# tobwei/APTAI

Hardware: AMD Instinct MI355X
Metric: utterances/sec (10 s @ 16 kHz) train-step (higher is better)
Workload: dtype bf16

## Files before the change

aptai_amd/_lib.py:

```python
from __future__ import annotations

import ctypes
import os
import subprocess
import threading

import torch

_HERE = os.path.dirname(os.path.abspath(__file__))
CSRC = os.path.join(_HERE, "csrc")
LIB_PATH = os.environ.get("APTAI_HIP_LIB") or os.path.join(CSRC, "libaptai_hip.so")

_lib = None
_lock = threading.Lock()

_P, _I64, _I, _F, _U64 = ctypes.c_void_p, ctypes.c_int64, ctypes.c_int, ctypes.c_float, ctypes.c_uint64
ARGTYPES = {
    "aptai_layernorm_fwd": [_P, _P, _P, _P, _P, _P, _I64, _I64, _F, _I, _P],
    "aptai_layernorm_bwd": [_P, _P, _P, _P, _P, _P, _P, _P, _F, _U64, _P, _P, _P, _I64, _I64, _P, _P],
    "aptai_layernorm_bwd_workspace_bytes": [_I64, _I64],
    "aptai_layernorm_bwd_finalize_multi": [_P, _I64, _I64, _P],
    "aptai_layernorm_fwd_f32in": [_P, _P, _P, _P, _P, _I64, _I64, _F, _P],
    "aptai_layernorm_fwd_f32in_split": [_P, _P, _P, _P, _P, _I, _I64, _I64, _F, _P],
    "aptai_attention_fwd": [_P, _P, _P, _P, _P, _I64, _I64, _I64, _I64, _F, _F, _U64, _I, _P],
    "aptai_attention_bwd": [_P, _P, _P, _P, _P, _P, _P, _P, _I64, _I64, _I64, _I64, _F, _F, _U64, _I, _I, _P],
    "aptai_attention_probs_fwd": [_P, _P, _P, _P, _I64, _I64, _I64, _I64, _F, _F, _U64, _I, _P],
    "aptai_attention_probs_bwd": [_P, _P, _P, _P, _P, _P, _I64, _I64, _I64, _I64, _F, _F, _U64, _I, _I, _P],
    "aptai_cast_f32_to_bf16": [_P, _P, _I64, _I64, _I64, _P],
    "aptai_conv_weight_to_bf16": [_P, _P, _I64, _I64, _I64, _P],
    "aptai_posconv_weight": [_P, _P, _P, _P, _P, _I64, _I64, _I64, _P],
    "aptai_posconv_pack": [_P, _P, _P, _P, _I64, _I64, _I64, _I64, _I64, _P],
    "aptai_frame_mask_fwd": [_P, _P, _P, _P, _I64, _I64, _I64, _I64, _P],
    "aptai_frame_mask_bwd": [_P, _P, _P, _P, _P, _I64, _I64, _I64, _I64, _P],
    "aptai_frame_mask_bwd_workspace_bytes": [_I64, _I64, _I64],
    "aptai_colsum_bf16": [_P, _I64, _P, _P, _I64, _I64, _I, _P],
    "aptai_colsum_workspace_bytes": [_I64, _I64],
    "aptai_dropout_bf16": [_P, _P, _I64, _F, _U64, _P],
    "aptai_dgelu_bf16": [_P, _P, _P, _I64, _P],
    "aptai_conv0_fwd": [_P, _I64, _I64, _P, _P, _P, _P, _I, _F, _P, _I64, _I64, _I64, _I64, _I64, _P, _P, _P],
    "aptai_conv0_bwd": [_P, _I64, _I64, _P, _P, _P, _P, _I, _F, _P, _I64, _I64, _P, _P, _P, _P, _P, _P, _P],
    "aptai_conv0_bwd_workspace_bytes": [_I64, _I64],
    "aptai_conv0_bwd_data": [_P, _I64, _I64, _P, _P, _P, _P, _I, _F, _P, _I64, _I64, _P, _P, _P, _P],
    "aptai_conv0_bwd_data_workspace_bytes": [_I64, _I64],
    "aptai_conv0_workspace_bytes": [_I64, _I64],
    "aptai_head_act_fwd": [_P, _P, _P, _I64, _F, _F, _U64, _P],
    "aptai_head_act_bwd": [_P, _P, _P, _P, _I64, _F, _F, _U64, _P],
    "aptai_lowpass_fir": [_P, _I64, _I64, _P, _I64, _P, _I64, _I64, _I, _I64, _I64, _I64, _I64, _I64, _P],
    "aptai_aptai_loss_fwd": [_P, _P, _P, _I64, _I64, _P, _I64, _I64, _I64, _I64, _F, _F, _P, _P, _P, _P],
    "aptai_aptai_loss_bwd": [_P, _P, _P, _I64, _I64, _P, _I64, _I64, _I64, _I64, _F, _F, _P, _P, _P, _P, _I64, _P],
    "aptai_aptai_loss_workspace_bytes": [],
    "aptai_gemm_workspace_bytes": [_I64, _I64, _I],
    "aptai_gemm_sk_workspace_bytes": [],
    "aptai_gemm_sk_status": [_P, _P, _P],
    "aptai_cast_multi": [_P, _I64, _I64, _P],
    "aptai_posconv_weight_bwd": [_P, _P, _P, _P, _P, _P, _P, _I64, _I64, _I64, _P],
    "aptai_spec_augment_mask": [_P, _P, _I64, _I64, _F, _I64, _I64, _U64, _P],
    "aptai_posconv_wgrad": [_P, _P, _P, _I64, _I64, _I64, _I64, _I64, _I64, _P],
    "aptai_posconv_gemm": [_P, _I64, _P, _P, _P, _P, _P, _I64, _I64, _I64, _I64, _I64, _I64, _I, _P],
    "aptai_adam_multi": [_P, _P, _I64, _I64, _F, _F, _F, _F, _F, _P],
    "aptai_sgemm_f32": [_P, _I, _I64, _I64, _P, _I64, _I64, _P, _I64, _P, _F, _I, _I64, _I64, _I64, _I64, _I64, _I64, _I64, _I64, _P, _P],
    "aptai_sgemm_workspace_bytes": [_I64, _I64, _I64, _I64],
    "aptai_colsum_f32_workspace_bytes": [_I64],
    "aptai_embed_pe_fwd": [_P, _P, _P, _P, _I64, _I64, _I64, _F, _U64, _P],
    "aptai_embed_bwd": [_P, _P, _P, _I64, _I64, _F, _U64, _P],
    "aptai_xattn_softmax_fwd": [_P, _P, _P, _P, _P, _P, _P, _I64, _I64, _I64, _P],
    "aptai_xattn_softmax_bwd": [_P, _P, _P, _P, _I64, _P, _I64, _I64, _P],
    "aptai_layernorm_f32_fwd": [_P, _P, _P, _P, _P, _P, _I64, _I64, _F, _P],
    "aptai_layernorm_f32_bwd": [_P, _P, _P, _P, _P, _P, _P, _P, _P, _I64, _I64, _P],
    "aptai_layernorm_f32_bwd_workspace_bytes": [_I64],
    "aptai_lstm_fwd": [_P, _P, _P, _P, _P, _P, _P, _I64, _I64, _I64, _I64, _P],
    "aptai_lstm_bwd": [_P, _P, _P, _P, _P, _P, _P, _I64, _I64, _I64, _I64, _P],
    "aptai_lstm_workspace_bytes": [_I64],
    "aptai_lstm_fwd_serial": [_P, _P, _P, _P, _P, _P, _I64, _I64, _I64, _I64, _P],
    "aptai_lstm_bwd_serial": [_P, _P, _P, _P, _P, _P, _I64, _I64, _I64, _I64, _P],
    "aptai_gather_alignment": [_P, _P, _P, _P, _I64, _I64, _I64, _P],
    "aptai_tanh_dropout_f32": [_P, _P, _P, _P, _I64, _F, _U64, _P],
    "aptai_dropout_f32": [_P, _P, _I64, _F, _U64, _P],
    "aptai_colsum_f32": [_P, _I64, _P, _P, _I64, _I64, _P],
    "aptai_ctc_fwd": [_P, _I64, _I64, _P, _I64, _P, _P, _P, _I64, _I64, _I64, _I, _I, _I, _P, _P, _P, _P, _I, _P],
    "aptai_ctc_bwd": [_P, _I64, _I64, _P, _I64, _P, _P, _P, _I64, _I64, _I64, _I, _I, _I, _P, _P, _P, _F, _P, _I64, _I, _I, _P],
    "aptai_ctc_workspace_bytes": [_I64, _I64, _I64],
    "aptai_ctc_viterbi": [_P, _I64, _I64, _P, _I64, _P, _P, _P, _I64, _I64, _I64, _I, _I, _P, _P, _P, _P, _P, _P],
    "aptai_ctc_viterbi_workspace_bytes": [_I64, _I64, _I64],
    "aptai_ctc_greedy_decode": [_P, _I64, _I64, _I64, _I64, _I64, _I, _P, _I64, _P, _P],
    "aptai_mx_quantize_bf16": [_P, _I64, _P, _I64, _P, _I64, _I64, _I64, _P],
    "aptai_gemm_mxfp8": [_P, _P, _I64, _I64, _P, _P, _I64, _I64, _P, _I64, _P, _I, _P, _I64, _I64, _I64, _I64, _P],
    "aptai_layernorm_fwd_mx": [_P, _P, _P, _P, _P, _I64, _P, _I64, _I64, _I64, _F, _P],
    "aptai_gemm_mxfp8_mxout": [_P, _P, _I64, _I64, _P, _P, _I64, _I64, _P, _I64, _P, _I64, _P, _I, _I64, _I64, _I64, _P],
    "aptai_split_f32": [_P, _I64, _I64, _I64, _I, _I, _I, _P, _I64, _P],
    "aptai_bias_act_res_f32": [_P, _I64, _P, _P, _I64, _P, _I64, _I64, _I64, _I, _P, _I64, _P],
    "aptai_softmax_rows_f32": [_P, _P, _I64, _I64, _I64, _P],
    "aptai_softmax_split_f32": [_P, _P, _I64, _I64, _I64, _I, _P, _I64, _P],
    "aptai_attention_exact_fwd": [_P, _I64, _P, _P, _I64, _I64, _I64, _I64, _I64, _I, _F, _P],
    "aptai_conv0_fwd_f32": [_P, _I64, _I64, _P, _P, _P, _P, _I, _F, _P, _I64, _I64, _P, _P],
    "aptai_conv0_fwd_split": [_P, _I64, _I64, _P, _P, _P, _P, _I, _F, _P, _I, _I64, _I64, _P, _P],
    "aptai_device_check": [ctypes.c_char_p, _I],
    "aptai_set_seed_salt": [_P, _P],
    "aptai_set_frame_bounds": [_P, _P],
}


class AptaiHipError(RuntimeError):
    pass


def build(force: bool = False, jobs: int = 8) -> str:
# ... 43 lines not shown
```

aptai_amd/csrc/gemm.hip:

```cpp
#include <stdlib.h>

#include <mutex>
#include <set>

#include "common.h"
#include "gemm_common.h"

using namespace aptai_gemm;

namespace {

#ifdef APTAI_STAMPS
__device__ unsigned long long g_stamps[4096 * 8];
#define APTAI_STAMP(slot)                                                                          \
    do {                                                                                           \
        if (threadIdx.x == 0 && blockIdx.x < 4096 && blockIdx.y == 0 && blockIdx.z == 0)           \
            g_stamps[blockIdx.x * 8 + (slot)] = wall_clock64();                                    \
    } while (0)
extern "C" int aptai_debug_read_stamps(void* host_out) {
    return hipMemcpyFromSymbol(host_out, HIP_SYMBOL(g_stamps), sizeof(g_stamps)) == hipSuccess ? 0 : 1;
}
#else
#define APTAI_STAMP(slot) do {} while (0)
#endif

void epi_trace(const GemmArgs& g, int tile) {
    static const bool on = getenv("APTAI_EPI_TRACE") != nullptr;
    if (!on) return;
    static std::mutex mu;
    static std::set<int> seen;
    const int w = g.flags | (g.out_pre ? EPX_PRE : 0) | (g.colscale_n > 0 ? EPX_CS : 0);
    std::lock_guard<std::mutex> lk(mu);
    if (!seen.insert(w).second) return;
    bool listed = false;
#define APTAI_EPI_CASE(W) listed = listed || (w == (W));
    APTAI_EPI_WORDS(APTAI_EPI_CASE)
#undef APTAI_EPI_CASE
    fprintf(stderr, "[aptai epi] flag word 0x%x (tile %d, %d x %d x %d): %s\n", w, tile, g.M, g.N, g.K, listed ? "compiled" : "RUN-TIME form");
}

template <bool A_KM, bool B_KM, bool OUT_F32, int BM_T = 128>
__device__ __forceinline__ void gemm_tile_body(GemmArgs g, const int bid, const int batch, const int split) {
    extern __shared__ __attribute__((aligned(16))) char smem[];
    APTAI_STAMP(0);
    const int tid = threadIdx.x;
    const int lane = tid & 63;
    const int wave = __builtin_amdgcn_readfirstlane(tid >> 6);
    const int wm = wave >> 1, wn = wave & 1;

    int tile_m, tile_n;
    raster2d(bid, g.tiles_m, g.tiles_n, g.raster_gm, tile_m, tile_n);
    constexpr int NI = BM_T / 32;
    constexpr int WM = BM_T / 2;
    constexpr int NA_IT = BM_T / 32;
    constexpr int A_BYTES_T = BM_T * BK * 2;
    constexpr int STAGE_T = A_BYTES_T + BN * BK * 2;
    constexpr int NPASS = BM_T / 16;
    static_assert(BM_T == 128 || (BM_T == 64 && !A_KM), "64-row tiles are built for K-contiguous A only");
    constexpr bool RING5 = A_KM && B_KM && BM_T == 128 && APTAI_GEMM_RING5;
// ... 316 lines not shown
                const int m = m0_e + pass * 16 + (tid_e >> 4);
                const bool ok = n_ok && m < g.M;
                u32x4 rq = {0u, 0u, 0u, 0u}, aq = {0u, 0u, 0u, 0u};
                if (ok && (flags & APTAI_EPI_RESIDUAL)) rq = *(const u32x4*)(g.residual + (long)m * g.ldr + n);
                if (ok && (flags & (APTAI_EPI_DGELU | APTAI_EPI_MUL_AUX))) aq = *(const u32x4*)(g.aux + (long)m * g.ldaux + n);
                one_pass(pass, aq, rq);
            }
        } else {
#pragma unroll
            for (int pass = 0; pass < NPASS; ++pass) {
                one_pass(pass, auxv[PREF ? pass : 0], resv[PREF ? pass : 0]);
                asm volatile("" ::: "memory");
            }
        }
    };
    if (OUT_F32) body(EpiWord<-1>{});
    else epi_dispatch(fx, body);
    APTAI_STAMP(3);
#ifdef APTAI_STAMPS
    asm volatile("s_waitcnt vmcnt(0)" ::: "memory");
    APTAI_STAMP(4);
#endif
}

template <bool A_KM, bool B_KM, bool OUT_F32>
__global__ __launch_bounds__(NTHREADS, 3) void gemm_kernel(GemmArgs g) {
#ifdef APTAI_EXP_STAGGER
    if (g.exp_sleep > 0) {
        bool late = true;
        if (g.exp_cu_count != nullptr) {
            unsigned hwid, xcc;
            asm volatile("s_getreg_b32 %0, hwreg(HW_REG_HW_ID)" : "=s"(hwid));
            asm volatile("s_getreg_b32 %0, hwreg(HW_REG_XCC_ID)" : "=s"(xcc));
            __shared__ unsigned arrival;
            if (threadIdx.x == 0) arrival = atomicAdd(g.exp_cu_count + ((xcc & 7u) * 256u + ((hwid >> 8) & 0xffu)), 1u);
            __syncthreads();
            late = arrival == 1u;
        }
        if (late) for (int i = 0; i < g.exp_sleep; ++i) __builtin_amdgcn_s_sleep(31);
    }
#endif
    gemm_tile_body<A_KM, B_KM, OUT_F32>(g, xcd_remap(blockIdx.x, g.tiles_m * g.tiles_n), gridDim.y > 1 ? (int)blockIdx.y : -1,
                                        blockIdx.z);
}

constexpr int SMEM_M64_BYTES = 2 * (64 + BN) * BK * 2;
template <bool B_KM, bool OUT_F32>
__global__ __launch_bounds__(NTHREADS, 3) void gemm_kernel_m64(GemmArgs g) {
    gemm_tile_body<false, B_KM, OUT_F32, 64>(g, xcd_remap(blockIdx.x, g.tiles_m * g.tiles_n), gridDim.y > 1 ? (int)blockIdx.y : -1,
                                             blockIdx.z);
}

constexpr int MAX_GROUP = 8;
struct GroupArgs {
    GemmArgs p[MAX_GROUP];
    int tile_end[MAX_GROUP];
    int n, total;
};

template <bool A_KM, bool B_KM, bool OUT_F32>
__global__ __launch_bounds__(NTHREADS, 3) void gemm_grouped_kernel(GroupArgs ga) {
    const int bid = xcd_remap(blockIdx.x, ga.total);
    int pi = 0;
#pragma unroll
    for (int i = 1; i < MAX_GROUP; ++i)
        if (i < ga.n && bid >= ga.tile_end[i - 1]) pi = i;
    const int first = pi ? ga.tile_end[pi - 1] : 0;
    gemm_tile_body<A_KM, B_KM, OUT_F32>(ga.p[pi], bid - first, -1, 0);
}

__global__ void splitk_reduce_kernel(const float* __restrict__ slabs, float* __restrict__ out, long n4, long slab_stride4,
                                     int nsplit, int accumulate) {
    const long stride = (long)gridDim.x * blockDim.x;
    for (long i = (long)blockIdx.x * blockDim.x + threadIdx.x; i < n4; i += stride) {
        f32x4 s = accumulate ? ((const f32x4*)out)[i] : (f32x4){0.f, 0.f, 0.f, 0.f};
        for (int k = 0; k < nsplit; ++k) s += ((const f32x4*)slabs)[(long)k * slab_stride4 + i];
        ((f32x4*)out)[i] = s;
    }
}

template <bool B_KM, bool OUT_F32>
int launch_gemm_m64(GemmArgs g, int nbatch, int nsplit, hipStream_t stream) {
    auto kern = gemm_kernel_m64<B_KM, OUT_F32>;
    g.tiles_m = (int)ceil_div(g.M, 64);
    dim3 grid(g.tiles_m * g.tiles_n, nbatch, nsplit);
    APTAI_LAUNCH(kern, grid, dim3(NTHREADS), SMEM_M64_BYTES, stream, g);
    APTAI_CHECK_LAUNCH("gemm_kernel_m64");
    return APTAI_OK;
}

template <bool A_KM, bool B_KM, bool OUT_F32>
int launch_gemm(const GemmArgs& g, int nbatch, int nsplit, hipStream_t stream) {
    auto kern = gemm_kernel<A_KM, B_KM, OUT_F32>;
    constexpr int smem = smem_for<A_KM, B_KM>();
    static bool attr_set = false;
    if (!attr_set) {
        (void)hipFuncSetAttribute((const void*)kern, hipFuncAttributeMaxDynamicSharedMemorySize, smem);
        attr_set = true;
    }
    dim3 grid(g.tiles_m * g.tiles_n, nbatch, nsplit);
#ifdef APTAI_EXP_STAGGER
    {
        GemmArgs ge = g;
        const char* e = getenv("APTAI_EXP_SLEEP");
        ge.exp_sleep = e ? atoi(e) : 0;
        const char* c = getenv("APTAI_EXP_CU_COUNT");
        ge.exp_cu_count = c ? (unsigned*)(uintptr_t)strtoull(c, nullptr, 10) : nullptr;
        const char* m = getenv("APTAI_EXP_SMEM");
        const int sm = m ? atoi(m) : smem;
        (void)hipFuncSetAttribute((const void*)kern, hipFuncAttributeMaxDynamicSharedMemorySize, sm > smem ? sm : smem);
        APTAI_LAUNCH(kern, grid, dim3(NTHREADS), sm > smem ? sm : smem, stream, ge);
        APTAI_CHECK_LAUNCH("gemm_kernel");
        return APTAI_OK;
    }
#endif
    APTAI_LAUNCH(kern, grid, dim3(NTHREADS), smem, stream, g);
    APTAI_CHECK_LAUNCH("gemm_kernel");
    return APTAI_OK;
}


// ... 775 lines not shown
            if (flags & APTAI_EPI_BIAS) {
                const f32x4 b0 = *(const f32x4*)(g.bias + n), b1 = *(const f32x4*)(g.bias + n + 4);
    #pragma unroll
                for (int r = 0; r < 4; ++r) { v[r] = fmaf(v[r], alpha, b0[r]); v[4 + r] = fmaf(v[4 + r], alpha, b1[r]); }
            } else if (flags & APTAI_EPI_ALPHA) {
    #pragma unroll
                for (int r = 0; r < 8; ++r) v[r] *= alpha;
            }
            if (OUT_F32) {
                if (flags & APTAI_EPI_RESIDUAL_F32) {
                    const float* R = (const float*)g.residual + (long)m * g.ldr + n;
                    const f32x4 r0 = *(const f32x4*)R, r1 = *(const f32x4*)(R + 4);
    #pragma unroll
                    for (int r = 0; r < 4; ++r) { v[r] += r0[r]; v[4 + r] += r1[r]; }
                }
                if (flags & APTAI_EPI_BIAS_ROW) { const float bm = g.bias[m];
#pragma unroll
                    for (int r = 0; r < 8; ++r) v[r] += bm; }
                if (flags & APTAI_EPI_SPLIT_OUT) { split_out_store(g, flags, v, (long)m, n); continue; }
                float* C = (float*)g.C + (long)split * g.slab_stride + (long)m * g.ldc + n;
                *(f32x4*)C = (f32x4){v[0], v[1], v[2], v[3]};
                *(f32x4*)(C + 4) = (f32x4){v[4], v[5], v[6], v[7]};
                continue;
            }
            epilogue_chunk<FM>(v, g, flags, (long)m, n, auxv[pass], resv[pass], sd0, sd1);
            __builtin_amdgcn_sched_barrier(0);
        }
    };
    if (OUT_F32) body(EpiWord<-1>{});
    else epi_dispatch(fx, body);
    APTAI_STAMP(3);
#ifdef APTAI_STAMPS
    asm volatile("s_waitcnt vmcnt(0)" ::: "memory");
    APTAI_STAMP(4);
#endif
}

template <bool A_KM, bool B_KM, bool OUT_F32>
int launch_gemm192(GemmArgs g, int nbatch, int nsplit, hipStream_t stream) {
    auto kern = gemm192_kernel<A_KM, B_KM, OUT_F32>;
    static bool attr_set = false;
    if (!attr_set) {
        (void)hipFuncSetAttribute((const void*)kern, hipFuncAttributeMaxDynamicSharedMemorySize, T3_SMEM);
        attr_set = true;
    }
    g.tiles_m = (int)ceil_div(g.M, T3_BM);
    g.tiles_n = (int)ceil_div(g.N, T3_BN);
    dim3 grid(g.tiles_m * g.tiles_n, nbatch, nsplit);
    APTAI_LAUNCH(kern, grid, dim3(T3_THREADS), T3_SMEM, stream, g);
    APTAI_CHECK_LAUNCH("gemm192_kernel");
    return APTAI_OK;
}

}

static int build_args(const aptai_gemm_desc* d, GemmArgs& g, int& nbatch, int& nsplit, const void* stream) {
    APTAI_REQUIRE(d != nullptr, "aptai_gemm_bf16: null descriptor");
    APTAI_REQUIRE(d->M > 0 && d->N > 0 && d->K > 0, "aptai_gemm_bf16: empty problem M=%ld N=%ld K=%ld", (long)d->M,
                  (long)d->N, (long)d->K);
    APTAI_REQUIRE(d->K % BK == 0, "aptai_gemm_bf16: K=%ld must be a multiple of %d", (long)d->K, BK);
    APTAI_REQUIRE(d->N % 8 == 0, "aptai_gemm_bf16: N=%ld must be a multiple of 8", (long)d->N);
    APTAI_REQUIRE(d->A && d->B && d->C, "aptai_gemm_bf16: null operand");
    APTAI_REQUIRE(d->lda % 8 == 0 && d->ldb % 8 == 0 && d->ldc % 8 == 0, "aptai_gemm_bf16: leading dims must keep 16-B alignment");
    if (d->residual) APTAI_REQUIRE(d->ldr % 8 == 0 && (uintptr_t)d->residual % 16 == 0, "aptai_gemm_bf16: residual must be 16-B aligned");
    if (d->aux) APTAI_REQUIRE(d->ldaux % 8 == 0 && (uintptr_t)d->aux % 16 == 0, "aptai_gemm_bf16: aux must be 16-B aligned");
    if (d->bias) APTAI_REQUIRE((uintptr_t)d->bias % 16 == 0, "aptai_gemm_bf16: bias must be 16-B aligned");
    APTAI_REQUIRE(((uintptr_t)d->A % 16 == 0) && ((uintptr_t)d->B % 16 == 0) && ((uintptr_t)d->C % 16 == 0),
                  "aptai_gemm_bf16: operands must be 16-byte aligned");
    if (d->a_kmajor) APTAI_REQUIRE(d->M % 8 == 0 && d->M >= 8, "aptai_gemm_bf16: K-major A needs M %% 8 == 0");
    if (d->b_kmajor) APTAI_REQUIRE(d->N >= 8, "aptai_gemm_bf16: K-major B needs N >= 8");
    if (d->flags & APTAI_EPI_BIAS) APTAI_REQUIRE(d->bias != nullptr, "aptai_gemm_bf16: EPI_BIAS without bias");
    if (d->flags & APTAI_EPI_RESIDUAL) APTAI_REQUIRE(d->residual != nullptr, "aptai_gemm_bf16: EPI_RESIDUAL without residual");
    if (d->flags & APTAI_EPI_RESIDUAL_F32)
        APTAI_REQUIRE(d->residual != nullptr && d->out_f32 && !(d->flags & APTAI_EPI_RESIDUAL) && d->split_k <= 1 && !d->accumulate &&
                      (d->tile == 128 || d->tile == 64 || d->tile == 192 || d->tile == 256 || d->tile == 257),
                      "aptai_gemm_bf16: EPI_RESIDUAL_F32 needs fp32 output, a residual, no split-K / accumulate and an explicit tile");
    if (d->flags & (APTAI_EPI_DGELU | APTAI_EPI_MUL_AUX)) APTAI_REQUIRE(d->aux != nullptr, "aptai_gemm_bf16: EPI_DGELU / EPI_MUL_AUX without aux");
    if (d->flags & APTAI_EPI_PRE_DGELU) APTAI_REQUIRE(d->out_pre != nullptr && (d->flags & APTAI_EPI_GELU), "aptai_gemm_bf16: EPI_PRE_DGELU needs EPI_GELU and out_pre");

    if (d->flags & APTAI_EPI_BIAS_ROW)
        APTAI_REQUIRE(d->out_f32 && d->bias != nullptr && !(d->flags & APTAI_EPI_BIAS) && (d->tile == 128 || d->tile == 192 || d->tile == 256) &&
                      d->split_k <= 1 && !d->accumulate, "aptai_gemm_bf16: EPI_BIAS_ROW needs out_f32, a bias of length M, no EPI_BIAS, tile 128 / 192 / 256");
    if (d->flags & APTAI_EPI_SPLIT_OUT)
        APTAI_REQUIRE(d->out_f32 && (d->tile == 128 || d->tile == 192 || d->tile == 256) && !d->a_kmajor && d->split_k <= 1 && !d->accumulate && (d->split_out_pieces == 3 || d->split_out_pieces == 6) &&
                      d->ldc >= d->split_out_pieces * d->N && d->N % 8 == 0,
                      "aptai_gemm_bf16: EPI_SPLIT_OUT needs out_f32, tile 128 / 192 / 256, 3 or 6 pieces and ldc >= pieces * N (bf16 elements)");
    APTAI_REQUIRE(d->colscale_n >= 0 && d->colscale_n % 8 == 0 && d->colscale_n <= d->N && (d->colscale_n == 0 || !d->out_f32),
                  "aptai_gemm_bf16: colscale_n must be a multiple of 8 within N, bf16 output only");
    memset(&g, 0, sizeof(g));
    g.A = (const bf16_t*)d->A; g.lda = d->lda;
    g.B = (const bf16_t*)d->B; g.ldb = d->ldb;
    g.C = d->C; g.ldc = d->ldc;
    g.M = (int)d->M; g.N = (int)d->N; g.K = (int)d->K;
    g.bias = d->bias;
    g.residual = (const bf16_t*)d->residual; g.ldr = d->ldr;
    g.out_pre = (bf16_t*)d->out_pre;
    g.aux = (const bf16_t*)d->aux; g.ldaux = d->ldaux;
    g.flags = d->flags;
    g.seed0 = (uint32_t)d->seed; g.seed1 = (uint32_t)(d->seed >> 32);
    g.salt = aptai_seed_salt(stream);
    g.thr16 = drop_thr16(d->dropout_p);
    g.dscale = drop_scale(g.thr16);
    if (g.thr16 == 0) g.flags &= ~APTAI_EPI_DROPOUT;
    g.alpha = d->alpha;
    g.colscale_n = d->colscale_n; g.colscale = d->colscale;
    g.split_pieces = d->split_out_pieces;
    g.split_bcol = (d->flags & APTAI_EPI_SPLIT_OUT) ? d->split_out_bcol : 0;
    g.hash_ld = d->N; g.hash_n0 = 0;
    g.tiles_m = (int)ceil_div(d->M, BM);
    g.tiles_n = (int)ceil_div(d->N, BN);
    {
        static int raster = -2;
        if (raster == -2) {
            const char* e = getenv("APTAI_GEMM_RASTER");
            raster = e ? atoi(e) : -1;
        }
        g.raster_gm = raster;
    }
    const int total_kt = g.K / BK;
    nsplit = d->split_k > 0 ? d->split_k : 1;
    if (nsplit > total_kt) nsplit = total_kt;
    g.ktiles_per_split = (int)ceil_div(total_kt, nsplit);
    nsplit = (int)ceil_div(total_kt, g.ktiles_per_split);

    nbatch = 1;
    g.nb_inner = 1;
    if (d->batch_outer > 1 || d->batch_inner > 1) {
        const int bo = d->batch_outer > 0 ? d->batch_outer : 1, bi = d->batch_inner > 0 ? d->batch_inner : 1;
        nbatch = bo * bi;
        g.nb_inner = bi;
        for (int l = 0; l < 2; ++l) {
            g.sA[l] = d->batch_stride_a[l]; g.sB[l] = d->batch_stride_b[l]; g.sC[l] = d->batch_stride_c[l];
            g.sBias[l] = d->batch_stride_bias[l]; g.sR[l] = d->batch_stride_res[l]; g.sAux[l] = d->batch_stride_aux[l];
            APTAI_REQUIRE(g.sA[l] % 8 == 0 && g.sB[l] % 8 == 0 && g.sC[l] % 8 == 0 && g.sBias[l] % 4 == 0 &&
                              g.sR[l] % 8 == 0 && g.sAux[l] % 8 == 0,
                          "aptai_gemm_bf16: batch strides must keep vector alignment");
        }
        APTAI_REQUIRE(nbatch <= 65535, "aptai_gemm_bf16: too many batches");
    }
    const bool f32 = d->out_f32 != 0;
    if (nbatch > 1) APTAI_REQUIRE(!(f32 && (d->split_k > 1 || d->accumulate)), "aptai_gemm_bf16: batched GEMM cannot split-K/accumulate");
    if (!f32) APTAI_REQUIRE(nsplit == 1, "aptai_gemm_bf16: split-K needs fp32 output");
    if (f32 && (nsplit > 1 || d->accumulate)) {
        APTAI_REQUIRE(d->workspace != nullptr, "aptai_gemm_bf16: split-K / accumulate needs a workspace");
        APTAI_REQUIRE(d->ldc == d->N, "aptai_gemm_bf16: split-K output must be dense (ldc == N)");
        APTAI_REQUIRE((size_t)d->workspace_bytes >= (size_t)nsplit * d->M * d->N * 4, "aptai_gemm_bf16: workspace too small");
        g.C = d->workspace;
        g.slab_stride = (long)d->M * d->N;
    }
    return APTAI_OK;
}

static int gemm_bf16_one(const aptai_gemm_desc* d, void* stream_, long hash_ld, int hash_n0);

extern "C" int aptai_gemm_bf16(const aptai_gemm_desc* d, void* stream_) {
    static const bool split_on = getenv("APTAI_GEMM_SPLITN") && atoi(getenv("APTAI_GEMM_SPLITN")) != 0;
    if (split_on && d != nullptr && d->tile == 0 && !d->out_f32 && !d->a_kmajor && d->split_k <= 1 && !d->accumulate && d->batch_outer <= 1 &&
        d->batch_inner <= 1 && d->colscale_n == 0 && d->sk_workspace == nullptr && d->M % 256 == 0 && d->N % 256 == 0 && d->K <= 1024 &&
        getenv("APTAI_GEMM_TILE") == nullptr) {
        const long tm = d->M / 256, tn = d->N / 256, T = tm * tn;
        if (T > 256 && T % 256 == 128 && (T - 128) % tm == 0) {
            const long n1 = (T - 128) / tm * 256, rem = d->N - n1;
            if ((d->M / 128) * (rem / 128) <= 512) {
                aptai_gemm_desc a = *d, b = *d;
                a.N = n1; a.tile = 256;
                b.N = rem; b.tile = 128;
                b.B = (const char*)d->B + (d->b_kmajor ? n1 * 2 : n1 * d->ldb * 2);
                b.C = (char*)d->C + n1 * 2;
                if (d->out_pre) b.out_pre = (char*)d->out_pre + n1 * 2;
                if (d->bias) b.bias = d->bias + n1;
                if (d->residual) b.residual = (const char*)d->residual + n1 * 2;
// ... 58 lines not shown
    }
    const bool sk_ok = d->sk_workspace != nullptr && d->sk_workspace_bytes >= sk_workspace_bytes() && nbatch == 1 && nsplit == 1 &&
                       !d->accumulate && d->M >= T2_BM && d->N >= T2_BN;
    if (tile == 257) APTAI_REQUIRE(sk_ok, "aptai_gemm_bf16: tile 257 (stream-K) needs sk_workspace (aptai_gemm_sk_workspace_bytes), no batching / "
                                          "split-K / accumulate and M, N >= 256");
    if (tile == 64 && d->a_kmajor) tile = 128;
    if (g.raster_gm < 0) g.raster_gm = 8;
    static const bool epi_runtime = getenv("APTAI_EPI_RUNTIME") && atoi(getenv("APTAI_EPI_RUNTIME")) != 0;
    if (epi_runtime) g.flags |= EPX_RUNTIME;
    if (!f32) epi_trace(g, tile);
    int rc;
    if (tile == 257) {
        if (!d->a_kmajor && !d->b_kmajor) rc = f32 ? launch_gemm256_sk<false, false, true>(g, d->sk_workspace, stream) : launch_gemm256_sk<false, false, false>(g, d->sk_workspace, stream);
        else if (!d->a_kmajor && d->b_kmajor) rc = f32 ? launch_gemm256_sk<false, true, true>(g, d->sk_workspace, stream) : launch_gemm256_sk<false, true, false>(g, d->sk_workspace, stream);
        else if (d->a_kmajor && d->b_kmajor) rc = f32 ? launch_gemm256_sk<true, true, true>(g, d->sk_workspace, stream) : launch_gemm256_sk<true, true, false>(g, d->sk_workspace, stream);
        else APTAI_FAIL(APTAI_ERR_INVALID, "aptai_gemm_bf16: A K-major with B K-contiguous is not built");
    } else
    if (tile == 64) {
        if (!d->b_kmajor) rc = f32 ? launch_gemm_m64<false, true>(g, nbatch, nsplit, stream) : launch_gemm_m64<false, false>(g, nbatch, nsplit, stream);
        else rc = f32 ? launch_gemm_m64<true, true>(g, nbatch, nsplit, stream) : launch_gemm_m64<true, false>(g, nbatch, nsplit, stream);
    } else
    if (tile == 448) {
        APTAI_REQUIRE(!f32 && !d->a_kmajor && nbatch == 1 && nsplit == 1 && !d->accumulate,
                      "aptai_gemm_bf16: tile 448 (256 x 192) is built for bf16 output, K-contiguous A, no batching / split-K");
        rc = launch_gemm_t4(g, d->b_kmajor != 0, stream);
    } else
    if (tile == 192) {
        if (!d->a_kmajor && !d->b_kmajor) rc = f32 ? launch_gemm192<false, false, true>(g, nbatch, nsplit, stream) : launch_gemm192<false, false, false>(g, nbatch, nsplit, stream);
        else if (!d->a_kmajor && d->b_kmajor) rc = f32 ? launch_gemm192<false, true, true>(g, nbatch, nsplit, stream) : launch_gemm192<false, true, false>(g, nbatch, nsplit, stream);
        else if (d->a_kmajor && d->b_kmajor) rc = f32 ? launch_gemm192<true, true, true>(g, nbatch, nsplit, stream) : launch_gemm192<true, true, false>(g, nbatch, nsplit, stream);
        else APTAI_FAIL(APTAI_ERR_INVALID, "aptai_gemm_bf16: A K-major with B K-contiguous is not built");
    } else
    if (tile == 256) {
        if (!d->a_kmajor && !d->b_kmajor) rc = f32 ? launch_gemm256<false, false, true>(g, nbatch, nsplit, stream) : launch_gemm256<false, false, false>(g, nbatch, nsplit, stream);
        else if (!d->a_kmajor && d->b_kmajor) rc = f32 ? launch_gemm256<false, true, true>(g, nbatch, nsplit, stream) : launch_gemm256<false, true, false>(g, nbatch, nsplit, stream);
        else if (d->a_kmajor && d->b_kmajor) rc = f32 ? launch_gemm256<true, true, true>(g, nbatch, nsplit, stream) : launch_gemm256<true, true, false>(g, nbatch, nsplit, stream);
        else APTAI_FAIL(APTAI_ERR_INVALID, "aptai_gemm_bf16: A K-major with B K-contiguous is not built");
    } else
    if (!d->a_kmajor && !d->b_kmajor) rc = f32 ? launch_gemm<false, false, true>(g, nbatch, nsplit, stream) : launch_gemm<false, false, false>(g, nbatch, nsplit, stream);
    else if (!d->a_kmajor && d->b_kmajor) rc = f32 ? launch_gemm<false, true, true>(g, nbatch, nsplit, stream) : launch_gemm<false, true, false>(g, nbatch, nsplit, stream);
    else if (d->a_kmajor && d->b_kmajor) rc = f32 ? launch_gemm<true, true, true>(g, nbatch, nsplit, stream) : launch_gemm<true, true, false>(g, nbatch, nsplit, stream);
    else APTAI_FAIL(APTAI_ERR_INVALID, "aptai_gemm_bf16: A K-major with B K-contiguous is not built");
    if (rc != APTAI_OK) return rc;
    if (f32 && (nsplit > 1 || d->accumulate)) {
        const long n4 = (long)d->M * d->N / 4;
        int blocks = (int)(n4 / 256 < 2048 ? (n4 + 255) / 256 : 2048);
        APTAI_LAUNCH(splitk_reduce_kernel, dim3(blocks), dim3(256), 0, stream, (const float*)d->workspace, final_out,
                           n4, g.slab_stride / 4, nsplit, d->accumulate ? 1 : 0);
        APTAI_CHECK_LAUNCH("splitk_reduce_kernel");
    }
    return APTAI_OK;
}

extern "C" int aptai_gemm_bf16_grouped(const aptai_gemm_desc* descs, int n, void* stream_) {
    hipStream_t stream = (hipStream_t)stream_;
    APTAI_REQUIRE(descs != nullptr && n >= 1 && n <= MAX_GROUP, "aptai_gemm_bf16_grouped: need 1..%d problems, got %d", MAX_GROUP, n);
    GroupArgs ga;
    memset(&ga, 0, sizeof(ga));
    int total = 0;
    for (int i = 0; i < n; ++i) {
        const aptai_gemm_desc* d = descs + i;
        int nbatch = 1, nsplit = 1;
        const int brc = build_args(d, ga.p[i], nbatch, nsplit, stream_);
        if (brc != APTAI_OK) return brc;
        if (ga.p[i].raster_gm < 0) ga.p[i].raster_gm = (d->a_kmajor && d->b_kmajor) ? 8 : 0;
        APTAI_REQUIRE(nbatch == 1 && nsplit == 1 && !d->accumulate, "aptai_gemm_bf16_grouped: problem %d: no batching, split-K or accumulate", i);
        APTAI_REQUIRE(d->a_kmajor == descs[0].a_kmajor && d->b_kmajor == descs[0].b_kmajor && (d->out_f32 != 0) == (descs[0].out_f32 != 0),
                      "aptai_gemm_bf16_grouped: problem %d: all problems must share the operand layout and output type", i);
        total += ga.p[i].tiles_m * ga.p[i].tiles_n;
        ga.tile_end[i] = total;
    }
    ga.n = n;
    ga.total = total;
    const bool f32 = descs[0].out_f32 != 0, akm = descs[0].a_kmajor != 0, bkm = descs[0].b_kmajor != 0;
    APTAI_REQUIRE(!(akm && !bkm), "aptai_gemm_bf16_grouped: A K-major with B K-contiguous is not built");
#define APTAI_GROUPED(AK, BK_, F)                                                                                      \
    do {                                                                                                              \
        auto kern = gemm_grouped_kernel<AK, BK_, F>;                                                                  \
        constexpr int smem = smem_for<AK, BK_>();                                                                     \
        static bool attr_set = false;                                                                                 \
        if (!attr_set) {                                                                                              \
            (void)hipFuncSetAttribute((const void*)kern, hipFuncAttributeMaxDynamicSharedMemorySize, smem);                  \
            attr_set = true;                                                                                          \
        }                                                                                                             \
        APTAI_LAUNCH(kern, dim3(total), dim3(NTHREADS), smem, stream, ga);                                            \
    } while (0)
    if (!akm && !bkm) { if (f32) APTAI_GROUPED(false, false, true); else APTAI_GROUPED(false, false, false); }
    else if (!akm && bkm) { if (f32) APTAI_GROUPED(false, true, true); else APTAI_GROUPED(false, true, false); }
    else { if (f32) APTAI_GROUPED(true, true, true); else APTAI_GROUPED(true, true, false); }
#undef APTAI_GROUPED
    APTAI_CHECK_LAUNCH("gemm_grouped_kernel");
    return APTAI_OK;
}

extern "C" int64_t aptai_gemm_sk_workspace_bytes(void) { return sk_workspace_bytes(); }

extern "C" int aptai_gemm_sk_status(void* sk_workspace, void* stream, int* status_out) {
    APTAI_REQUIRE(sk_workspace != nullptr && status_out != nullptr, "aptai_gemm_sk_status: null pointer");
    unsigned v = 0;
    if (hipMemcpyAsync(&v, sk_workspace, 4, hipMemcpyDeviceToHost, (hipStream_t)stream) != hipSuccess ||
        hipStreamSynchronize((hipStream_t)stream) != hipSuccess)
        APTAI_FAIL(APTAI_ERR_LAUNCH, "aptai_gemm_sk_status: reading the status word failed");
    if (v != 0 && hipMemsetAsync(sk_workspace, 0, 4, (hipStream_t)stream) != hipSuccess)
        APTAI_FAIL(APTAI_ERR_LAUNCH, "aptai_gemm_sk_status: clearing the status word failed");
    *status_out = (int)v;
    return APTAI_OK;
}

extern "C" int64_t aptai_gemm_workspace_bytes(int64_t M, int64_t N, int split_k) {
    return (int64_t)(split_k > 0 ? split_k : 1) * M * N * 4;
}
```

include/aptai_hip.h:

```cpp
#ifndef APTAI_HIP_H
#define APTAI_HIP_H
#include <stdint.h>

#ifdef __cplusplus
extern "C" {
#endif

typedef enum {
    APTAI_OK = 0,
    APTAI_ERR_INVALID = -1,
    APTAI_ERR_LAUNCH = -2,
    APTAI_ERR_NO_DEVICE = -3
} aptai_status;

const char* aptai_last_error(void);
int aptai_version(void);
int aptai_device_check(char* name, int name_len);
int aptai_set_seed_salt(void* stream, const void* device_ptr_2xu32);
int aptai_set_frame_bounds(void* stream, const void* device_ptr_2xi32);

enum {
    APTAI_EPI_BIAS = 1,
    APTAI_EPI_GELU = 2,
    APTAI_EPI_RESIDUAL = 4,
    APTAI_EPI_DROPOUT = 8,
    APTAI_EPI_DGELU = 16,
    APTAI_EPI_ALPHA = 32,
    APTAI_EPI_PRE_DGELU = 64,
    APTAI_EPI_MUL_AUX = 128,
    APTAI_EPI_RESIDUAL_F32 = 256,
    APTAI_EPI_BIAS_ROW = 1024,
    APTAI_EPI_SPLIT_OUT = 512
};

typedef struct {
    const void* A; int64_t lda;
    const void* B; int64_t ldb;
    void* C; int64_t ldc;
    int64_t M, N, K;
    int a_kmajor, b_kmajor, out_f32;
    int flags;
    const float* bias;
    const void* residual; int64_t ldr;
    void* out_pre;
    const void* aux; int64_t ldaux;
    float alpha;
    float dropout_p; uint64_t seed;
    int split_k;
    int accumulate;
    void* workspace; int64_t workspace_bytes;
    int batch_outer, batch_inner;
    int64_t batch_stride_a[2], batch_stride_b[2], batch_stride_c[2], batch_stride_bias[2], batch_stride_res[2],
        batch_stride_aux[2];
    int tile;
    int colscale_n; float colscale;
    void* sk_workspace;
    int64_t sk_workspace_bytes;
    int split_out_pieces;
    int split_out_bcol;
} aptai_gemm_desc;

int aptai_gemm_bf16(const aptai_gemm_desc* desc, void* stream);
int aptai_gemm_bf16_grouped(const aptai_gemm_desc* descs, int n, void* stream);
int64_t aptai_gemm_workspace_bytes(int64_t M, int64_t N, int split_k);
int64_t aptai_gemm_sk_workspace_bytes(void);
int aptai_gemm_sk_status(void* sk_workspace, void* stream, int* status_out);

int aptai_split_f32(const float* x, int64_t ldx, int64_t rows, int64_t cols, int pattern, int pieces, int act, void* out, int64_t ldo,
                    void* stream);
int aptai_bias_act_res_f32(const float* x, int64_t ldx, const float* bias, const float* res, int64_t ldr, float* y, int64_t ldy,
                           int64_t rows, int64_t cols, int act, const int32_t* lens, int64_t rows_per_b, void* stream);
int aptai_softmax_rows_f32(float* s, const int32_t* lens, int64_t B, int64_t heads, int64_t Tp, void* stream);
int aptai_softmax_split_f32(const float* s, const int32_t* lens, int64_t B, int64_t heads, int64_t Tp, int pieces, void* out, int64_t ldo,
                            void* stream);
int aptai_attention_exact_fwd(const void* qkv_split, int64_t ld, const int32_t* lens, void* ctx_split, int64_t ldo, int64_t B, int64_t Tp,
                              int64_t H, int64_t heads, int pieces, float scale, void* stream);
int aptai_conv0_fwd_f32(const float* audio, int64_t B, int64_t S, const float* weight, const float* bias, const float* gamma,
                        const float* beta, int mode, float eps, float* out, int64_t T_real, int64_t T_alloc, const float* stats,
                        void* stream);
int aptai_conv0_fwd_split(const float* audio, int64_t B, int64_t S, const float* weight, const float* bias, const float* gamma,
                          const float* beta, int mode, float eps, void* out_split, int pieces, int64_t T_real, int64_t T_alloc,
                          const float* stats, void* stream);

int aptai_layernorm_fwd(const void* x, const float* gamma, const float* beta, void* y, float* mean, float* rstd,
                        int64_t rows, int64_t cols, float eps, int gelu_after, void* stream);
int aptai_layernorm_fwd_f32in(const float* x, const float* gamma, const float* beta, void* y_bf16, float* y_f32, int64_t rows,
                              int64_t cols, float eps, void* stream);
int aptai_layernorm_fwd_f32in_split(const float* x, const float* gamma, const float* beta, float* y_f32, void* y_split, int pieces,
                                    int64_t rows, int64_t cols, float eps, void* stream);
int aptai_layernorm_bwd(const void* dy, const void* x, const float* mean, const float* rstd, const float* gamma,
                        const void* dres, void* dx, void* dx_drop, float dropout_p, uint64_t seed, float* dgamma,
                        float* dbeta, void* workspace, int64_t rows, int64_t cols, const float* beta_if_gelu_after,
                        void* stream);
int64_t aptai_layernorm_bwd_workspace_bytes(int64_t rows, int64_t cols);
int aptai_layernorm_bwd_finalize_multi(const int64_t* table_dev, int64_t njobs, int64_t max_cols, void* stream);

int aptai_attention_fwd(const void* qkv, const int32_t* lens, void* ctx, float* lse2, float* ctx_f32, int64_t B, int64_t Tp,
                        int64_t H, int64_t heads, float scale, float dropout_p, uint64_t seed, int q_prescaled, void* stream);
int aptai_attention_bwd(const void* qkv, const int32_t* lens, const void* ctx, const float* ctx_f32, const void* dctx,
                        const float* lse2, float* delta_ws, void* dqkv, int64_t B, int64_t Tp, int64_t H, int64_t heads, float scale,
                        float dropout_p, uint64_t seed, int dctx_zero_beyond_len, int q_prescaled, void* stream);

int aptai_attention_probs_fwd(const void* qkv, const int32_t* lens, const float* lse2, float* probs, int64_t B, int64_t Tp, int64_t H,
                              int64_t heads, float scale, float dropout_p, uint64_t seed, int q_prescaled, void* stream);
int aptai_attention_probs_bwd(const void* qkv, const int32_t* lens, const float* lse2, const float* dprobs, float* rowsum_ws, void* dqkv,
                              int64_t B, int64_t Tp, int64_t H, int64_t heads, float scale, float dropout_p, uint64_t seed,
                              int q_prescaled, int accumulate, void* stream);

int aptai_cast_f32_to_bf16(const float* src, void* dst, int64_t rows, int64_t cols, int64_t ld_dst, void* stream);
int aptai_cast_multi(const int64_t* table_dev, int64_t njobs, int64_t max_n, void* stream);
int aptai_adam_multi(const int64_t* table_dev, const int64_t* dyn_dev, int64_t njobs, int64_t max_n, float lr, float beta1,
                     float beta2, float eps, float weight_decay, void* stream);
int aptai_conv_weight_to_bf16(const float* src, void* dst, int64_t N, int64_t C, int64_t Kw, void* stream);
int aptai_posconv_weight(const float* v, const float* gain, float* norm_ws, void* w_fwd, void* w_dgrad, int64_t H,
                         int64_t groups, int64_t Kw, void* stream);
int aptai_posconv_weight_bwd(const float* dw_fwd, const float* v, const float* gain, const float* norm, float* dv, float* dgain,
// ... 120 lines not shown
```

Measured before the change: 1715.

## Plan XCD-aware tile-to-run assignment for grouped GEMM to improve L2 panel reuse

Adds a host-side planner that assigns tiles from grouped GEMM problems to the 8 XCD runs (blockIdx & 7), greedily grouping tiles so each XCD touches fewer distinct A/B panels. It also co-locates dependent small problems with their parent's rows and keeps load balanced within a quota. The plan is cached per problem shape and pointer identity and decoded per block in the kernel, which replaces the arithmetic xcd_remap and raster. The cost is some idle padding blocks and plan lookup overhead on the host, and the scheme depends on blocks being dispatched round-robin across XCDs.

```diff
diff --git a/aptai_amd/_lib.py b/aptai_amd/_lib.py
--- a/aptai_amd/_lib.py
+++ b/aptai_amd/_lib.py
@@ -52,6 +52,7 @@
     "aptai_gemm_workspace_bytes": [_I64, _I64, _I],
     "aptai_gemm_sk_workspace_bytes": [],
     "aptai_gemm_sk_status": [_P, _P, _P],
+    "aptai_gemm_grouped_plan": [_P, _I, _P, _P, _P],
     "aptai_cast_multi": [_P, _I64, _I64, _P],
     "aptai_posconv_weight_bwd": [_P, _P, _P, _P, _P, _P, _P, _I64, _I64, _I64, _P],
     "aptai_spec_augment_mask": [_P, _P, _I64, _I64, _F, _I64, _I64, _U64, _P],
diff --git a/aptai_amd/csrc/gemm.hip b/aptai_amd/csrc/gemm.hip
--- a/aptai_amd/csrc/gemm.hip
+++ b/aptai_amd/csrc/gemm.hip
@@ -3,8 +3,12 @@
 #include <mutex>
 #include <set>
 
+#include <map>
+#include <vector>
+
 #include "common.h"
 #include "gemm_common.h"
+#include "grouped_plan.h"
 
 using namespace aptai_gemm;
 
@@ -427,21 +431,48 @@
 }
 
 constexpr int MAX_GROUP = 8;
+static_assert(MAX_GROUP == aptai_plan::MAX_PROB, "the plan indexes the same problem list");
 struct GroupArgs {
     GemmArgs p[MAX_GROUP];
     int tile_end[MAX_GROUP];
     int n, total;
+    aptai_plan::Plan plan;
 };
+static_assert(sizeof(GroupArgs) <= 4096, "GroupArgs travels as a kernel argument");
 
 template <bool A_KM, bool B_KM, bool OUT_F32>
 __global__ __launch_bounds__(NTHREADS, 3) void gemm_grouped_kernel(GroupArgs ga) {
-    const int bid = xcd_remap(blockIdx.x, ga.total);
-    int pi = 0;
-#pragma unroll
-    for (int i = 1; i < MAX_GROUP; ++i)
-        if (i < ga.n && bid >= ga.tile_end[i - 1]) pi = i;
-    const int first = pi ? ga.tile_end[pi - 1] : 0;
-    gemm_tile_body<A_KM, B_KM, OUT_F32>(ga.p[pi], bid - first, -1, 0);
+    int pi = 0, bid;
+    const bool planned = ga.plan.nseg > 0;
+    if (planned) {
+        const int run = blockIdx.x & 7, idx = blockIdx.x >> 3;
+        if (idx >= (int)ga.plan.run_len[run]) {
+#ifdef APTAI_STAMPS
+            if (threadIdx.x == 0 && blockIdx.x < 4096) g_stamps[blockIdx.x * 8] = g_stamps[blockIdx.x * 8 + 4] = 0;
+#endif
+            return;
+        }
+        int tile_m, tile_n;
+        aptai_plan::plan_decode(ga.plan, run, idx, pi, tile_m, tile_n);
+        bid = tile_m * ga.p[pi].tiles_n + tile_n;
+    } else {
+        bid = xcd_remap(blockIdx.x, ga.total);
+#pragma unroll
+        for (int i = 1; i < MAX_GROUP; ++i)
+            if (i < ga.n && bid >= ga.tile_end[i - 1]) pi = i;
+        bid -= pi ? ga.tile_end[pi - 1] : 0;
+    }
+#ifdef APTAI_STAMPS
+    if (threadIdx.x == 0 && blockIdx.x < 4096) {
+        unsigned xcc;
+        asm volatile("s_getreg_b32 %0, hwreg(HW_REG_XCC_ID)" : "=s"(xcc));
+        g_stamps[blockIdx.x * 8 + 5] = xcc & 7u;
+        g_stamps[blockIdx.x * 8 + 6] = (unsigned long long)pi;
+    }
+#endif
+    GemmArgs g = ga.p[pi];
+    if (planned) g.raster_gm = 0;
+    gemm_tile_body<A_KM, B_KM, OUT_F32>(g, bid, -1, 0);
 }
 
 __global__ void splitk_reduce_kernel(const float* __restrict__ slabs, float* __restrict__ out, long n4, long slab_stride4,
@@ -1323,6 +1354,15 @@
     return APTAI_OK;
 }
 
+}
+
+static int raster_env() {
+    static int raster = -2;
+    if (raster == -2) {
+        const char* e = getenv("APTAI_GEMM_RASTER");
+        raster = e ? atoi(e) : -1;
+    }
+    return raster;
 }
 
 static int build_args(const aptai_gemm_desc* d, GemmArgs& g, int& nbatch, int& nsplit, const void* stream) {
@@ -1380,14 +1420,7 @@
     g.hash_ld = d->N; g.hash_n0 = 0;
     g.tiles_m = (int)ceil_div(d->M, BM);
     g.tiles_n = (int)ceil_div(d->N, BN);
-    {
-        static int raster = -2;
-        if (raster == -2) {
-            const char* e = getenv("APTAI_GEMM_RASTER");
-            raster = e ? atoi(e) : -1;
-        }
-        g.raster_gm = raster;
-    }
+    g.raster_gm = raster_env();
     const int total_kt = g.K / BK;
     nsplit = d->split_k > 0 ? d->split_k : 1;
     if (nsplit > total_kt) nsplit = total_kt;
@@ -1552,18 +1585,84 @@
     return APTAI_OK;
 }
 
+static aptai_plan::Prob plan_prob(const aptai_gemm_desc* d) {
+    aptai_plan::Prob p;
+    p.A = d->A; p.lda = (long)d->lda;
+    p.B = d->B; p.ldb = (long)d->ldb;
+    p.K = (int)d->K;
+    p.tiles_m = (int)ceil_div(d->M, BM);
+    p.tiles_n = (int)ceil_div(d->N, BN);
+    p.raster_gm = raster_env() < 0 ? ((d->a_kmajor && d->b_kmajor) ? 8 : 0) : raster_env();
+    p.half = d->M <= BM / 2;
+    return p;
+}
+
+static const aptai_plan::Plan& grouped_plan_cached(const aptai_plan::Prob* pr, int n) {
+    static std::mutex mu;
+    static std::map<std::vector<long>, aptai_plan::Plan> cache;
+    std::vector<long> key;
+    std::vector<std::pair<const void*, long>> seen;
+    auto ident = [&](const void* ptr, long ld) {
+        for (size_t i = 0; i < seen.size(); ++i)
+            if (seen[i] == std::make_pair(ptr, ld)) return (long)i;
+        seen.push_back(std::make_pair(ptr, ld));
+        return (long)seen.size() - 1;
+    };
+    for (int i = 0; i < n; ++i) {
+        const long item[] = {ident(pr[i].A, pr[i].lda), ident(pr[i].B, pr[i].ldb), pr[i].lda, pr[i].ldb, pr[i].K, pr[i].tiles_m, pr[i].tiles_n,
+                             pr[i].raster_gm, pr[i].half};
+        key.insert(key.end(), item, item + sizeof(item) / sizeof(item[0]));
+    }
+    std::lock_guard<std::mutex> lk(mu);
+    auto it = cache.find(key);
+    if (it == cache.end()) {
+        aptai_plan::Plan plan;
+        aptai_plan::make_plan(pr, n, plan);
+        it = cache.emplace(key, plan).first;
+    }
+    return it->second;
+}
+
+extern "C" int aptai_gemm_grouped_plan(const aptai_gemm_desc* descs, int n, int32_t* out_tile, int32_t* out_run_end, int* out_planned) {
+    APTAI_REQUIRE(descs != nullptr && n >= 1 && n <= MAX_GROUP, "aptai_gemm_grouped_plan: need 1..%d problems, got %d", MAX_GROUP, n);
+    APTAI_REQUIRE(out_tile != nullptr && out_run_end != nullptr, "aptai_gemm_grouped_plan: null output");
+    aptai_plan::Prob pr[MAX_GROUP];
+    for (int i = 0; i < n; ++i) {
+        APTAI_REQUIRE(descs[i].M > 0 && descs[i].N > 0 && descs[i].K > 0, "aptai_gemm_grouped_plan: problem %d is empty", i);
+        pr[i] = plan_prob(descs + i);
+    }
+    const aptai_plan::Plan& plan = grouped_plan_cached(pr, n);
+    std::vector<aptai_plan::Tile> runs[aptai_plan::N_RUN];
+    if (plan.nseg > 0) aptai_plan::plan_runs(plan, runs);
+    else aptai_plan::arith_runs(pr, n, runs);
+    int k = 0;
+    for (int r = 0; r < aptai_plan::N_RUN; ++r) {
+        for (const aptai_plan::Tile& t : runs[r]) {
+            out_tile[3 * k] = t.prob;
+            out_tile[3 * k + 1] = t.m;
+            out_tile[3 * k + 2] = t.n;
+            ++k;
+        }
+        out_run_end[r] = k;
+    }
+    if (out_planned) *out_planned = plan.nseg > 0 ? 1 : 0;
+    return APTAI_OK;
+}
+
 extern "C" int aptai_gemm_bf16_grouped(const aptai_gemm_desc* descs, int n, void* stream_) {
     hipStream_t stream = (hipStream_t)stream_;
     APTAI_REQUIRE(descs != nullptr && n >= 1 && n <= MAX_GROUP, "aptai_gemm_bf16_grouped: need 1..%d problems, got %d", MAX_GROUP, n);
     GroupArgs ga;
     memset(&ga, 0, sizeof(ga));
+    aptai_plan::Prob pr[MAX_GROUP];
     int total = 0;
     for (int i = 0; i < n; ++i) {
         const aptai_gemm_desc* d = descs + i;
         int nbatch = 1, nsplit = 1;
         const int brc = build_args(d, ga.p[i], nbatch, nsplit, stream_);
         if (brc != APTAI_OK) return brc;
-        if (ga.p[i].raster_gm < 0) ga.p[i].raster_gm = (d->a_kmajor && d->b_kmajor) ? 8 : 0;
+        pr[i] = plan_prob(d);
+        ga.p[i].raster_gm = pr[i].raster_gm;
         APTAI_REQUIRE(nbatch == 1 && nsplit == 1 && !d->accumulate, "aptai_gemm_bf16_grouped: problem %d: no batching, split-K or accumulate", i);
         APTAI_REQUIRE(d->a_kmajor == descs[0].a_kmajor && d->b_kmajor == descs[0].b_kmajor && (d->out_f32 != 0) == (descs[0].out_f32 != 0),
                       "aptai_gemm_bf16_grouped: problem %d: all problems must share the operand layout and output type", i);
@@ -1572,6 +1671,16 @@
     }
     ga.n = n;
     ga.total = total;
+    ga.plan = grouped_plan_cached(pr, n);
+#ifdef APTAI_STAMPS
+    if (getenv("APTAI_STAMPS_ARITH")) ga.plan.nseg = 0;
+#endif
+    int nblocks = total;
+    if (ga.plan.nseg > 0) {
+        int longest = 0;
+        for (int r = 0; r < aptai_plan::N_RUN; ++r) longest = ga.plan.run_len[r] > longest ? ga.plan.run_len[r] : longest;
+        nblocks = aptai_plan::N_RUN * longest;
+    }
     const bool f32 = descs[0].out_f32 != 0, akm = descs[0].a_kmajor != 0, bkm = descs[0].b_kmajor != 0;
     APTAI_REQUIRE(!(akm && !bkm), "aptai_gemm_bf16_grouped: A K-major with B K-contiguous is not built");
 #define APTAI_GROUPED(AK, BK_, F)                                                                                      \
@@ -1583,7 +1692,7 @@
             (void)hipFuncSetAttribute((const void*)kern, hipFuncAttributeMaxDynamicSharedMemorySize, smem);                  \
             attr_set = true;                                                                                          \
         }                                                                                                             \
-        APTAI_LAUNCH(kern, dim3(total), dim3(NTHREADS), smem, stream, ga);                                            \
+        APTAI_LAUNCH(kern, dim3(nblocks), dim3(NTHREADS), smem, stream, ga);                                          \
     } while (0)
     if (!akm && !bkm) { if (f32) APTAI_GROUPED(false, false, true); else APTAI_GROUPED(false, false, false); }
     else if (!akm && bkm) { if (f32) APTAI_GROUPED(false, true, true); else APTAI_GROUPED(false, true, false); }
diff --git a/aptai_amd/csrc/grouped_plan.h b/aptai_amd/csrc/grouped_plan.h
--- /dev/null
+++ b/aptai_amd/csrc/grouped_plan.h
@@ -0,0 +1,250 @@
+#pragma once
+#include <stdint.h>
+
+#include <algorithm>
+#include <set>
+#include <tuple>
+#include <vector>
+
+#ifdef __HIPCC__
+#define APTAI_PLAN_HD __host__ __device__ __forceinline__
+#else
+#define APTAI_PLAN_HD inline
+#endif
+
+namespace aptai_plan {
+
+constexpr int MAX_PROB = 8, N_RUN = 8, MAX_SEG = 64;
+constexpr int XCD_SLOTS = 64;
+
+struct Prob {
+    const void* A; long lda;
+    const void* B; long ldb;
+    int K;
+    int tiles_m, tiles_n;
+    int raster_gm;
+    int half;
+};
+
+struct Seg {
+    uint16_t start;
+    uint8_t prob, pad;
+    uint16_t m0, nm, n0;
+};
+struct Plan {
+    int nseg;
+    uint16_t run_len[N_RUN];
+    uint8_t seg_first[N_RUN + 1];
+    Seg seg[MAX_SEG];
+};
+
+APTAI_PLAN_HD void plan_decode(const Plan& p, int run, int idx, int& prob, int& tile_m, int& tile_n) {
+    int s = p.seg_first[run];
+    const int last = p.seg_first[run + 1] - 1;
+    while (s < last && (int)p.seg[s + 1].start <= idx) ++s;
+    const int r = idx - (int)p.seg[s].start, nm = p.seg[s].nm;
+    prob = p.seg[s].prob;
+    tile_m = (int)p.seg[s].m0 + r % nm;
+    tile_n = (int)p.seg[s].n0 + r / nm;
+}
+
+inline int arith_xcd_remap(int bid, int nwg) {
+    const int q = nwg >> 3, r = nwg & 7, xcd = bid & 7;
+    return (xcd < r ? xcd * (q + 1) : r * (q + 1) + (xcd - r) * q) + (bid >> 3);
+}
+inline void arith_raster2d(int bid, int tiles_m, int tiles_n, int gm, int& tile_m, int& tile_n) {
+    if (gm <= 1) { tile_m = bid / tiles_n; tile_n = bid % tiles_n; return; }
+    const int group = gm * tiles_n;
+    const int first = (bid / group) * gm;
+    const int rows = tiles_m - first < gm ? tiles_m - first : gm;
+    const int r = bid % group;
+    tile_m = first + r % rows;
+    tile_n = r / rows;
+}
+
+struct Tile { int prob, m, n; };
+typedef std::tuple<const void*, long, int, int> PanelKey;
+
+struct Score {
+    int over;
+    int max_panels;
+    int sum_panels;
+    int max_weight;
+    bool operator<(const Score& o) const {
+        return std::tie(over, max_panels, sum_panels, max_weight) < std::tie(o.over, o.max_panels, o.sum_panels, o.max_weight);
+    }
+};
+
+inline Score score_runs(const Prob* pr, const std::vector<Tile> (&runs)[N_RUN], int* panels_out = nullptr) {
+    Score s = {0, 0, 0, 0};
+    int total = 0, max_tiles = 0, sum_weight = 0;
+    for (int r = 0; r < N_RUN; ++r) {
+        std::set<PanelKey> seen;
+        int w = 0;
+        for (const Tile& t : runs[r]) {
+            const Prob& p = pr[t.prob];
+            seen.insert(PanelKey(p.A, p.lda, p.K, t.m));
+            seen.insert(PanelKey(p.B, p.ldb, p.K, t.n));
+            w += p.half ? 1 : 2;
+        }
+        const int np = (int)seen.size();
+        if (panels_out) panels_out[r] = np;
+        s.max_panels = std::max(s.max_panels, np);
+        s.sum_panels += np;
+        s.max_weight = std::max(s.max_weight, w);
+        sum_weight += w;
+        max_tiles = std::max(max_tiles, (int)runs[r].size());
+        total += (int)runs[r].size();
+    }
+    const int even = (sum_weight + N_RUN - 1) / N_RUN;
+    s.over = std::max(0, s.max_weight - (even + even / 8));
+    if (total <= N_RUN * XCD_SLOTS) s.over += std::max(0, max_tiles - XCD_SLOTS);
+    return s;
+}
+
+inline void arith_runs(const Prob* pr, int n, std::vector<Tile> (&runs)[N_RUN]) {
+    int total = 0;
+    for (int i = 0; i < n; ++i) total += pr[i].tiles_m * pr[i].tiles_n;
+    for (int r = 0; r < N_RUN; ++r) runs[r].clear();
+    for (int b = 0; b < total; ++b) {
+        int bid = arith_xcd_remap(b, total), pi = 0, first = 0;
+        while (bid - first >= pr[pi].tiles_m * pr[pi].tiles_n) first += pr[pi].tiles_m * pr[pi].tiles_n, ++pi;
+        Tile t = {pi, 0, 0};
+        arith_raster2d(bid - first, pr[pi].tiles_m, pr[pi].tiles_n, pr[pi].raster_gm, t.m, t.n);
+        runs[b & 7].push_back(t);
+    }
+}
+
+inline void plan_runs(const Plan& p, std::vector<Tile> (&runs)[N_RUN]) {
+    for (int r = 0; r < N_RUN; ++r) {
+        runs[r].clear();
+        for (int i = 0; i < (int)p.run_len[r]; ++i) {
+            Tile t;
+            plan_decode(p, r, i, t.prob, t.m, t.n);
+            runs[r].push_back(t);
+        }
+    }
+}
+
+struct Rect { int prob, m0, nm, n0, nn; };
+
+inline bool greedy_pass(const Prob* pr, int n, const int* parent, const std::vector<int>& order, int quota, int budget, Plan& out, bool& overflow) {
+    std::vector<Rect> rects[N_RUN];
+    std::set<PanelKey> panels[N_RUN];
+    int tiles[N_RUN] = {0};
+    int r = 0;
+    for (int i : order) {
+        const Prob& p = pr[i];
+        const bool along_n = p.tiles_m <= p.tiles_n;
+        const int line = along_n ? p.tiles_m : p.tiles_n, lines = along_n ? p.tiles_n : p.tiles_m;
+        int pos = 0;
+        while (pos < lines) {
+            int k = 0;
+            if (r == N_RUN - 1) k = lines - pos;
+            else {
+                std::set<PanelKey> trial = panels[r];
+                for (int j = 0; j < line; ++j) trial.insert(along_n ? PanelKey(p.A, p.lda, p.K, j) : PanelKey(p.B, p.ldb, p.K, j));
+                while (pos + k < lines && tiles[r] + (k + 1) * line <= quota) {
+                    trial.insert(along_n ? PanelKey(p.B, p.ldb, p.K, pos + k) : PanelKey(p.A, p.lda, p.K, pos + k));
+                    if ((int)trial.size() > budget) break;
+                    ++k;
+                }
+                if (k == 0 && tiles[r] == 0) k = 1;
+                if (k == 0) { ++r; continue; }
+            }
+            const Rect rc = along_n ? Rect{i, 0, line, pos, k} : Rect{i, pos, k, 0, line};
+            rects[r].push_back(rc);
+            for (int a = 0; a < rc.nm; ++a) panels[r].insert(PanelKey(p.A, p.lda, p.K, rc.m0 + a));
+            for (int b = 0; b < rc.nn; ++b) panels[r].insert(PanelKey(p.B, p.ldb, p.K, rc.n0 + b));
+            tiles[r] += k * line;
+            pos += k;
+        }
+    }
+    overflow = (int)panels[N_RUN - 1].size() > budget;
+    std::vector<std::vector<Rect>> extra[N_RUN];
+    for (int q = 0; q < N_RUN; ++q) extra[q].resize(rects[q].size());
+    for (int j = 0; j < n; ++j) {
+        if (parent[j] < 0) continue;
+        for (int c = 0; c < pr[j].tiles_n; ++c) {
+            int best_run = -1, best_rect = -1;
+            for (int q = 0; q < N_RUN; ++q)
+                for (int e = 0; e < (int)rects[q].size(); ++e) {
+                    const Rect& rc = rects[q][e];
+                    if (rc.prob == parent[j] && c >= rc.m0 && c < rc.m0 + rc.nm && (best_run < 0 || tiles[q] < tiles[best_run])) {
+                        best_run = q;
+                        best_rect = e;
+                    }
+                }
+            if (best_run < 0) return false;
+            std::vector<Rect>& ex = extra[best_run][best_rect];
+            if (!ex.empty() && ex.back().prob == j && ex.back().n0 + ex.back().nn == c) ++ex.back().nn;
+            else ex.push_back(Rect{j, 0, 1, c, 1});
+            ++tiles[best_run];
+        }
+    }
+    out.nseg = 0;
+    for (int q = 0; q < N_RUN; ++q) {
+        out.seg_first[q] = (uint8_t)out.nseg;
+        int start = 0;
+        auto emit = [&](const Rect& rc) {
+            if (out.nseg < MAX_SEG) out.seg[out.nseg] = Seg{(uint16_t)start, (uint8_t)rc.prob, 0, (uint16_t)rc.m0, (uint16_t)rc.nm, (uint16_t)rc.n0};
+            ++out.nseg;
+            start += rc.nm * rc.nn;
+        };
+        for (int e = 0; e < (int)rects[q].size(); ++e) {
+            emit(rects[q][e]);
+            for (const Rect& rc : extra[q][e]) emit(rc);
+        }
+        if (start > 0xffff) return false;
+        out.run_len[q] = (uint16_t)start;
+    }
+    out.seg_first[N_RUN] = (uint8_t)(out.nseg < 255 ? out.nseg : 255);
+    return out.nseg <= MAX_SEG;
+}
+
+inline void make_plan(const Prob* pr, int n, Plan& plan) {
+    plan = Plan();
+    if (n < 1 || n > MAX_PROB) return;
+    for (int i = 0; i < n; ++i)
+        if (pr[i].tiles_m > 0xffff || pr[i].tiles_n > 0xffff) return;
+    int parent[MAX_PROB];
+    for (int j = 0; j < n; ++j) {
+        parent[j] = -1;
+        if (pr[j].tiles_m != 1) continue;
+        for (int i = 0; i < n && parent[j] < 0; ++i)
+            if (i != j && pr[i].tiles_m > 1 && pr[i].A == pr[j].B && pr[i].lda == pr[j].ldb && pr[i].K == pr[j].K && pr[i].tiles_m == pr[j].tiles_n)
+                parent[j] = i;
+    }
+    std::vector<int> given, by_size;
+    int main_tiles = 0;
+    for (int i = 0; i < n; ++i)
+        if (parent[i] < 0) {
+            given.push_back(i);
+            main_tiles += pr[i].tiles_m * pr[i].tiles_n;
+        }
+    by_size = given;
+    std::stable_sort(by_size.begin(), by_size.end(), [&](int a, int b) { return pr[a].tiles_m * pr[a].tiles_n > pr[b].tiles_m * pr[b].tiles_n; });
+
+    std::vector<Tile> runs[N_RUN];
+    arith_runs(pr, n, runs);
+    const Score present = score_runs(pr, runs);
+    Score best = present;
+    const int q0 = (main_tiles + N_RUN - 1) / N_RUN;
+    for (int pass = 0; pass < (by_size == given ? 1 : 2); ++pass)
+        for (int quota = q0; quota <= q0 + q0 / 8 + 1; ++quota)
+            for (int budget = present.max_panels; budget >= 2; --budget) {
+                Plan trial;
+                bool overflow = false;
+                if (!greedy_pass(pr, n, parent, pass ? by_size : given, quota, budget, trial, overflow)) continue;
+                plan_runs(trial, runs);
+                const Score s = score_runs(pr, runs);
+                if (s < best) {
+                    best = s;
+                    plan = trial;
+                }
+                if (overflow) break;
+            }
+    if (!(std::tie(best.over, best.max_panels, best.sum_panels) < std::tie(present.over, present.max_panels, present.sum_panels))) plan.nseg = 0;
+}
+
+}
diff --git a/include/aptai_hip.h b/include/aptai_hip.h
--- a/include/aptai_hip.h
+++ b/include/aptai_hip.h
@@ -62,6 +62,7 @@
 
 int aptai_gemm_bf16(const aptai_gemm_desc* desc, void* stream);
 int aptai_gemm_bf16_grouped(const aptai_gemm_desc* descs, int n, void* stream);
+int aptai_gemm_grouped_plan(const aptai_gemm_desc* descs, int n, int32_t* out_tile, int32_t* out_run_end, int* out_planned);
 int64_t aptai_gemm_workspace_bytes(int64_t M, int64_t N, int split_k);
 int64_t aptai_gemm_sk_workspace_bytes(void);
 int aptai_gemm_sk_status(void* sk_workspace, void* stream, int* status_out);
```

Result: no change. 1725, median of 6 (+0.6%).
